# Dipet/pytorch_yolo

Measured on NVIDIA B200. Metric: YOLO decode+NMS images/sec, higher is better.
Workload: dtype f32

## Files before the change

pytorch_yolo_b200/csrc/decode.cu:

```cuda
#include <cuda.h>

#include "common.cuh"

namespace yb {

struct ScaleDev {
    const float* head;
    int ny, nx, na, row_off;
    int plane;
    int vec;
    int n_units;
    int first_block;
    int first_tile;
    int tiles_per_slab;
    float stride;
    float av[YOLO_B200_MAX_ANCHORS][2];
};

struct DecodeParams {
    ScaleDev sc[YOLO_B200_MAX_SCALES];
    int n_scales, batch, nc, rows_per_img;
    float conf, min_wh;
    yolo_b200_box* cand_box;
    yolo_b200_meta* cand_meta;
    int cap;
    int32_t* count;
    int32_t* overflow;
    float* io;
    int tp;
    int n_tiles;
    int use_tmap;
    alignas(64) CUtensorMap tmap[YOLO_B200_MAX_SCALES];
};

#ifndef YB_DC_THREADS
#define YB_DC_THREADS 128
#endif
#ifndef YB_DC_UNROLL
#define YB_DC_UNROLL 16
#endif
#ifndef YB_DC_UNROLL1
#define YB_DC_UNROLL1 40
#endif
#ifndef YB_DC_MINBLOCKS
#define YB_DC_MINBLOCKS 4
#endif
#ifndef YB_DC_SMEM_PAD
#define YB_DC_SMEM_PAD 0
#endif

constexpr int kDcThreads = YB_DC_THREADS;

template <int VEC>
__device__ __forceinline__ void load_vec(float (&dst)[VEC], const float* p) {
    if constexpr (VEC == 4) {
        const float4 v = ldg_stream4(p);
        dst[0] = v.x; dst[1] = v.y; dst[2] = v.z; dst[3] = v.w;
    } else {
        dst[0] = ldg_stream(p);
    }
}

__device__ __noinline__ void rescan_classes(const float* cls0, int stride, int nc, float& conf, int& cls) {
    float best = -1.0f;
    int bi = 0;
    for (int k = 0; k < nc; ++k) {
        const float s = sigmoidf_rn(cls0[(size_t)k * stride]);
        if (s > best) { best = s; bi = k; }
    }
    conf = best;
    cls = bi;
}

__device__ __forceinline__ void finish_anchor(const DecodeParams& P, const ScaleDev& S, bool active, int img, int a, int pos,
                                              float t0, float t1, float t2, float t3, float t4,
                                              float m, float m2, int idx, const float* cls0, int cls_stride) {
    const int nc = P.nc;
    const float stride = S.stride;
    const float conf = P.conf;
    const float kSlack = 1.00003f;
    bool emit = false;
    yolo_b200_box box = {0.f, 0.f, 0.f, 0.f};
    float score = 0.f, cls_conf = 1.0f;
    int cls = 0;
    if (active) {
        const float so = sigmoidf_rn(t4);
        const float sm = (nc > 1) ? sigmoidf_rn(m) : 1.0f;
        if (so * sm * kSlack > conf) {
            cls_conf = sm;
            cls = idx;
            if (nc > 1 && sigmoidf_rn(m2) * kSlack >= sm) rescan_classes(cls0, cls_stride, nc, cls_conf, cls);
            score = __fmul_rn(so, cls_conf);
            if (score > conf) {
                const float w = decode_wh(t2, S.av[a][0], stride);
                const float h = decode_wh(t3, S.av[a][1], stride);
                if (w > P.min_wh && h > P.min_wh && finitef(w) && finitef(h)) {
                    const int gy = pos / S.nx;
                    const int gx = pos - gy * S.nx;
                    const float x = decode_xy(t0, (float)gx, stride);
                    const float y = decode_xy(t1, (float)gy, stride);
                    if (finitef(x) && finitef(y)) {
                        emit = true;
                        box = to_corners(x, y, w, h);
                    }
                }
            }
        }
    }
    const int slot = warp_claim_slot(emit, img, P.count);
    if (emit) {
        if (slot < P.cap) {
            const int row = S.row_off + a * S.plane + pos;
            store_candidate(P.cand_box, P.cand_meta, (size_t)img * P.cap + slot, box, score, cls_conf, cls, row);
        } else {
            atomicMax(P.overflow, 1);
        }
    }
}

template <int VEC, int kDcUnroll>
__device__ __forceinline__ void decode_compact_body(const DecodeParams& P, const ScaleDev& S, int block_local) {
    const int nc = P.nc;
    const int no = nc + 5;
    const int plane = S.plane;
    const int pv_per_slab = plane / VEC;

    int unit = block_local * kDcThreads + (int)threadIdx.x;
    const bool active = unit < S.n_units;
    if (!active) unit = S.n_units - 1;
    const int slab = unit / pv_per_slab;
    const int pv = unit - slab * pv_per_slab;
    const int img = slab / S.na;
    const int a = slab - img * S.na;
    const int pos0 = pv * VEC;
    const float* base = S.head + (size_t)slab * no * plane + pos0;

    float t[5][VEC];
#pragma unroll
    for (int c = 0; c < 5; ++c) load_vec<VEC>(t[c], base + (size_t)c * plane);

    float m[VEC], m2[VEC];
    int idx[VEC];
#pragma unroll
    for (int j = 0; j < VEC; ++j) { m[j] = __int_as_float(0xff800000); m2[j] = m[j]; idx[j] = 0; }

    const float* cbase = base + (size_t)5 * plane;
    int c0 = 0;
    auto scan = [&](const float (&v)[kDcUnroll][VEC], int cfirst) {
#pragma unroll
        for (int u = 0; u < kDcUnroll; ++u) {
#pragma unroll
            for (int j = 0; j < VEC; ++j) {
                const float x = v[u][j];
                const bool up = x > m[j];
                m2[j] = up ? m[j] : fmaxf(m2[j], x);
                idx[j] = up ? (cfirst + u) : idx[j];
                m[j] = fmax_nan(m[j], x);
            }
        }
    };
    auto fetch = [&](float (&v)[kDcUnroll][VEC], int cfirst) {
#pragma unroll
        for (int u = 0; u < kDcUnroll; ++u) load_vec<VEC>(v[u], cbase + (size_t)(cfirst + u) * plane);
    };
    if (nc > 1) {
        for (; c0 + kDcUnroll <= nc; c0 += kDcUnroll) {
            float v[kDcUnroll][VEC];
            fetch(v, c0);
            scan(v, c0);
        }
        for (; c0 < nc; ++c0) {
            float v[VEC];
            load_vec<VEC>(v, cbase + (size_t)c0 * plane);
#pragma unroll
            for (int j = 0; j < VEC; ++j) {
                const float x = v[j];
                const bool up = x > m[j];
                m2[j] = up ? m[j] : fmaxf(m2[j], x);
                idx[j] = up ? c0 : idx[j];
                m[j] = fmax_nan(m[j], x);
            }
        }
    }

#pragma unroll
    for (int j = 0; j < VEC; ++j)
        finish_anchor(P, S, active, img, a, pos0 + j, t[0][j], t[1][j], t[2][j], t[3][j], t[4][j],
                      m[j], m2[j], idx[j], cbase + j, plane);
}


__global__ void __launch_bounds__(kDcThreads, YB_DC_MINBLOCKS)
decode_compact_kernel(const __grid_constant__ DecodeParams P) {
    int s = 0;
#pragma unroll
    for (int k = 1; k < YOLO_B200_MAX_SCALES; ++k)
        if (k < P.n_scales && (int)blockIdx.x >= P.sc[k].first_block) s = k;
    const ScaleDev& S = P.sc[s];
    const int block_local = (int)blockIdx.x - S.first_block;
    if (S.vec == 4) decode_compact_body<4, YB_DC_UNROLL>(P, S, block_local);
    else            decode_compact_body<1, YB_DC_UNROLL1>(P, S, block_local);
}

__device__ __forceinline__ uint32_t smem_u32(const void* p) { return (uint32_t)__cvta_generic_to_shared(p); }

__device__ __forceinline__ void mbar_init(uint64_t* bar, int count) {
    asm volatile("mbarrier.init.shared::cta.b64 [%0], %1;" ::"r"(smem_u32(bar)), "r"(count));
}
__device__ __forceinline__ void mbar_expect_tx(uint64_t* bar, uint32_t bytes) {
    asm volatile("mbarrier.arrive.expect_tx.shared::cta.b64 _, [%0], %1;" ::"r"(smem_u32(bar)), "r"(bytes) : "memory");
}
__device__ __forceinline__ void mbar_wait(uint64_t* bar, uint32_t phase) {
    asm volatile(
        "{\n\t.reg .pred p;\n\t"
        "WAIT_%=:\n\t"
        "mbarrier.try_wait.parity.shared::cta.b64 p, [%0], %1;\n\t"
        "@p bra DONE_%=;\n\t"
        "bra WAIT_%=;\n\t"
        "DONE_%=:\n\t}" ::"r"(smem_u32(bar)), "r"(phase) : "memory");
}
__device__ __forceinline__ void tma_bulk_g2s(void* dst, const void* src, uint32_t bytes, uint64_t* bar) {
    asm volatile("cp.async.bulk.shared::cluster.global.mbarrier::complete_tx::bytes [%0], [%1], %2, [%3];"
                 ::"r"(smem_u32(dst)), "l"(src), "r"(bytes), "r"(smem_u32(bar)) : "memory");
}


__device__ __forceinline__ void tma_tile_g2s(void* dst, const CUtensorMap* map, int x, int y, uint64_t* bar) {
    asm volatile("cp.async.bulk.tensor.2d.shared::cluster.global.tile.mbarrier::complete_tx::bytes [%0], [%1, {%2, %3}], [%4];"
                 ::"r"(smem_u32(dst)), "l"(map), "r"(x), "r"(y), "r"(smem_u32(bar)) : "memory");
}

constexpr int kTcConsumers = 256;
constexpr int kTcThreads = kTcConsumers + 32;
constexpr int kTcStages = 2;

__device__ __forceinline__ void mbar_arrive(uint64_t* bar) {
    asm volatile("mbarrier.arrive.shared::cta.b64 _, [%0];" ::"r"(smem_u32(bar)) : "memory");
}
__device__ __forceinline__ void consumer_bar_sync() {
    asm volatile("bar.sync 1, %0;" ::"n"(kTcConsumers) : "memory");
}

__global__ void __launch_bounds__(kTcThreads, 1)
decode_compact_tma_kernel(const __grid_constant__ DecodeParams P) {
    extern __shared__ __align__(128) float smem[];
    __shared__ __align__(8) uint64_t full[kTcStages];
    __shared__ __align__(8) uint64_t empty[kTcStages];
    const int tid = threadIdx.x;
    const int nc = P.nc, no = nc + 5, tp = P.tp;
    const int stage_floats = no * tp;

    if (tid == 0) {
#pragma unroll
        for (int s = 0; s < kTcStages; ++s) { mbar_init(&full[s], 1); mbar_init(&empty[s], kTcConsumers / 32); }
        asm volatile("fence.mbarrier_init.release.cluster;" ::: "memory");
    }
    __syncthreads();

    auto locate = [&](int tile, int& sc, int& slab, int& p0) {
        sc = 0;
#pragma unroll
        for (int k = 1; k < YOLO_B200_MAX_SCALES; ++k)
            if (k < P.n_scales && tile >= P.sc[k].first_tile) sc = k;
        const int local = tile - P.sc[sc].first_tile;
        slab = local / P.sc[sc].tiles_per_slab;
        p0 = (local - slab * P.sc[sc].tiles_per_slab) * tp;
    };

    if (tid >= kTcConsumers) {
        const int lane = tid & 31;
        int it = 0;
        for (int tile = blockIdx.x; tile < P.n_tiles; tile += gridDim.x, ++it) {
            const int st = it % kTcStages;
            mbar_wait(&empty[st], ((it / kTcStages) & 1) ^ 1);
            int sc, slab, p0;
            locate(tile, sc, slab, p0);
            const ScaleDev& S = P.sc[sc];
            if (S.vec != 4) continue;
            float* dst = smem + (size_t)st * stage_floats;
            if (P.use_tmap) {
                if (lane == 0) {
                    mbar_expect_tx(&full[st], (uint32_t)stage_floats * 4u);
                    tma_tile_g2s(dst, &P.tmap[sc], p0, slab * no, &full[st]);
                }
                continue;
            }
            const int np = min(tp, S.plane - p0);
            const uint32_t bytes = (uint32_t)np * 4u;
            if (lane == 0) mbar_expect_tx(&full[st], bytes * (uint32_t)no);
            __syncwarp();
            const float* src = S.head + (size_t)slab * no * S.plane + p0;
            for (int c = lane; c < no; c += 32)
                tma_bulk_g2s(dst + (size_t)c * tp, src + (size_t)c * S.plane, bytes, &full[st]);
        }
        return;
    }

    uint32_t full_parity = 0;
    int it = 0;
    for (int tile = blockIdx.x; tile < P.n_tiles; tile += gridDim.x, ++it) {
        const int st = it % kTcStages;
        int sc, slab, p0;
        locate(tile, sc, slab, p0);
        const ScaleDev& S = P.sc[sc];
        const int np = min(tp, S.plane - p0);
        float* tl = smem + (size_t)st * stage_floats;
        if (S.vec == 4) {
            mbar_wait(&full[st], (full_parity >> st) & 1u);
            full_parity ^= 1u << st;
        } else {
            consumer_bar_sync();
            const float* src = S.head + (size_t)slab * no * S.plane + p0;
            for (int c = tid >> 5; c < no; c += kTcConsumers / 32) {
                const float* row = src + (size_t)c * S.plane;
                float v[8];
#pragma unroll
                for (int k = 0; k < 8; ++k) { const int p = (tid & 31) + 32 * k; v[k] = p < np ? ldg_stream(row + p) : 0.0f; }
#pragma unroll
                for (int k = 0; k < 8; ++k) { const int p = (tid & 31) + 32 * k; if (p < np) tl[c * tp + p] = v[k]; }
            }
            consumer_bar_sync();
        }
        const bool active = tid < np;
        const int p = active ? tid : 0;
        const float* col = tl + p;
        const float t0 = col[0], t1 = col[tp], t2 = col[2 * tp], t3 = col[3 * tp], t4 = col[4 * tp];
        float m = __int_as_float(0xff800000), m2 = m;
        int idx = 0;
        const float* cls0 = col + 5 * tp;
        if (nc > 1) {
#pragma unroll 8
            for (int c = 0; c < nc; ++c) {
                const float x = cls0[c * tp];
                const bool up = x > m;
                m2 = up ? m : fmaxf(m2, x);
                idx = up ? c : idx;
                m = fmax_nan(m, x);
            }
        }
        const int img = slab / S.na;
        const int a = slab - img * S.na;
        finish_anchor(P, S, active, img, a, p0 + p, t0, t1, t2, t3, t4, m, m2, idx, cls0, tp);
        __syncwarp();
        if ((tid & 31) == 0) mbar_arrive(&empty[st]);
    }
}

constexpr int kDdPos = 128;
constexpr int kDdThreads = 256;
constexpr int kDdUnroll = 5;

__device__ __forceinline__ int dd_tiles_per_slab(int plane) { return (plane + kDdPos - 1) / kDdPos; }

__global__ void __launch_bounds__(kDdThreads)
decode_dense_kernel(const __grid_constant__ DecodeParams P) {
    extern __shared__ __align__(128) float smem[];
    int s = 0;
#pragma unroll
    for (int k = 1; k < YOLO_B200_MAX_SCALES; ++k)
        if (k < P.n_scales && (int)blockIdx.x >= P.sc[k].first_block) s = k;
    const ScaleDev& S = P.sc[s];
    const int nc = P.nc, no = nc + 5, plane = S.plane;
    const int tps = dd_tiles_per_slab(plane);
    const int block_local = (int)blockIdx.x - S.first_block;
    const int slab = block_local / tps;
    const int tile = block_local - slab * tps;
    const int img = slab / S.na;
    const int a = slab - img * S.na;
    const int p0 = tile * kDdPos;
    const int np = min(kDdPos, plane - p0);

    const size_t out_off = ((size_t)img * P.rows_per_img + S.row_off + (size_t)a * plane + p0) * no;
    const int mis = (int)(out_off & 3);
    float* tl = smem + mis;

    if (S.vec == 4) {
        const int warp = (int)threadIdx.x >> 5, lane = (int)threadIdx.x & 31, g = lane >> 3;
        if (4 * lane < np) {
            const float* src = S.head + (size_t)slab * no * plane + p0 + 4 * lane;
            const float stride = S.stride;
            float* drow[4];
#pragma unroll
            for (int k = 0; k < 4; ++k) drow[k] = tl + (4 * lane + ((k + g) & 3)) * no;
            auto put = [&](int ch, const float (&r)[4]) {
#pragma unroll
                for (int k = 0; k < 4; ++k) {
                    const float val = g == 0 ? r[k] : g == 1 ? r[(k + 1) & 3] : g == 2 ? r[(k + 2) & 3] : r[(k + 3) & 3];
                    drow[k][ch] = val;
                }
            };
            int c = warp;
            if (c < 4) {
                const float4 t = ldg_stream4(src + (size_t)c * plane);
                const float tv[4] = {t.x, t.y, t.z, t.w};
                float r[4];
#pragma unroll
                for (int j = 0; j < 4; ++j) {
                    const int pos = p0 + 4 * lane + j;
                    const int gy = pos / S.nx, gx = pos - gy * S.nx;
                    r[j] = c == 0 ? decode_xy(tv[j], (float)gx, stride)
                         : c == 1 ? decode_xy(tv[j], (float)gy, stride)
                                  : decode_wh(tv[j], S.av[a][c - 2], stride);
                }
                put(c, r);
                c += kDdThreads / 32;
            }
            const float* q = src + (size_t)c * plane;
            const size_t qstep = (size_t)(kDdThreads / 32) * plane;
            for (; c + (kDdUnroll - 1) * (kDdThreads / 32) < no; c += kDdUnroll * (kDdThreads / 32)) {
                float4 v[kDdUnroll];
#pragma unroll
                for (int u = 0; u < kDdUnroll; ++u, q += qstep) v[u] = ldg_stream4(q);
#pragma unroll
                for (int u = 0; u < kDdUnroll; ++u) {
                    const float r[4] = {sigmoidf_rn(v[u].x), sigmoidf_rn(v[u].y), sigmoidf_rn(v[u].z), sigmoidf_rn(v[u].w)};
                    put(c + u * (kDdThreads / 32), r);
                }
            }
            for (; c < no; c += kDdThreads / 32, q += qstep) {
                const float4 t = ldg_stream4(q);
                const float r[4] = {sigmoidf_rn(t.x), sigmoidf_rn(t.y), sigmoidf_rn(t.z), sigmoidf_rn(t.w)};
                put(c, r);
            }
            if (nc == 1 && warp == 5) {
                const float one[4] = {1.0f, 1.0f, 1.0f, 1.0f};
                put(5, one);
            }
        }
    } else {
        const int p = (int)threadIdx.x % kDdPos;
        const int half = (int)threadIdx.x / kDdPos;
        const int n_sig = no - 4;
        const int n0 = n_sig > 4 ? (n_sig - 4) / 2 : 0;
        if (p < np) {
            const float* src = S.head + (size_t)slab * no * plane + p0 + p;
            float* dst = tl + p * no;
            const float stride = S.stride;
            if (half == 0) {
                const int pos = p0 + p;
                const int gy = pos / S.nx, gx = pos - gy * S.nx;
                const float t0 = ldg_stream(src), t1 = ldg_stream(src + plane);
                const float t2 = ldg_stream(src + 2 * (size_t)plane), t3 = ldg_stream(src + 3 * (size_t)plane);
                dst[0] = decode_xy(t0, (float)gx, stride);
                dst[1] = decode_xy(t1, (float)gy, stride);
                dst[2] = decode_wh(t2, S.av[a][0], stride);
                dst[3] = decode_wh(t3, S.av[a][1], stride);
            }
            int c = half ? 4 + n0 : 4;
            const int c_end = half ? no : 4 + n0;
            const float* q = src + (size_t)c * plane;
            float* d = dst + c;
            for (; c + kDdUnroll <= c_end; c += kDdUnroll, d += kDdUnroll) {
                float v[kDdUnroll];
    #pragma unroll
                for (int u = 0; u < kDdUnroll; ++u, q += plane) v[u] = ldg_stream(q);
    #pragma unroll
                for (int u = 0; u < kDdUnroll; ++u) d[u] = sigmoidf_rn(v[u]);
            }
            for (; c < c_end; ++c, ++d, q += plane) *d = sigmoidf_rn(ldg_stream(q));
            if (nc == 1 && half == 1) dst[5] = 1.0f;
        }
    }
    __syncthreads();

    const int n_el = np * no;
    float* out = P.io + out_off;
    const int head = min(n_el, (4 - mis) & 3);
    if ((int)threadIdx.x < head) out[threadIdx.x] = tl[threadIdx.x];
    const int n4 = (n_el - head) >> 2;
    const float4* s4 = reinterpret_cast<const float4*>(tl + head);
    float4* o4 = reinterpret_cast<float4*>(out + head);
    for (int i = threadIdx.x; i < n4; i += kDdThreads) o4[i] = s4[i];
    const int done = head + (n4 << 2);
    if ((int)threadIdx.x < n_el - done) out[done + threadIdx.x] = tl[done + threadIdx.x];
}

struct DenseTmaParams {
    int stages_in, bufs_out;
};

__device__ __forceinline__ void bulk_s2g(void* gdst, const void* ssrc, uint32_t bytes) {
    asm volatile("cp.async.bulk.global.shared::cta.bulk_group [%0], [%1], %2;" ::"l"(gdst), "r"(smem_u32(ssrc)), "r"(bytes) : "memory");
}
__device__ __forceinline__ void bulk_commit() { asm volatile("cp.async.bulk.commit_group;" ::: "memory"); }
template <int N>
__device__ __forceinline__ void bulk_wait_read() { asm volatile("cp.async.bulk.wait_group.read %0;" ::"n"(N) : "memory"); }
__device__ __forceinline__ void fence_proxy_async_smem() { asm volatile("fence.proxy.async.shared::cta;" ::: "memory"); }

constexpr int kDtMaxStages = 4;

__global__ void __launch_bounds__(kTcThreads, 1)
decode_dense_tma_kernel(const __grid_constant__ DecodeParams P, const DenseTmaParams Q) {
    extern __shared__ __align__(128) float smem[];
    __shared__ __align__(8) uint64_t full[kDtMaxStages];
    __shared__ __align__(8) uint64_t empty[kDtMaxStages];
    const int tid = threadIdx.x;
    const int nc = P.nc, no = nc + 5;
    constexpr int tp = kDdPos;
    const int stage_floats = no * tp;
    const int out_floats = stage_floats + 4;
    float* out_base = smem + (size_t)Q.stages_in * stage_floats;

    if (tid == 0) {
        for (int s = 0; s < Q.stages_in; ++s) { mbar_init(&full[s], 1); mbar_init(&empty[s], kTcConsumers / 32); }
        asm volatile("fence.mbarrier_init.release.cluster;" ::: "memory");
    }
    __syncthreads();

    auto locate = [&](int tile, int& sc, int& slab, int& p0) {
        sc = 0;
#pragma unroll
        for (int k = 1; k < YOLO_B200_MAX_SCALES; ++k)
            if (k < P.n_scales && tile >= P.sc[k].first_tile) sc = k;
        const int local = tile - P.sc[sc].first_tile;
        slab = local / P.sc[sc].tiles_per_slab;
        p0 = (local - slab * P.sc[sc].tiles_per_slab) * tp;
    };

    if (tid >= kTcConsumers) {
        if ((tid & 31) != 0) return;
        int it = 0, st = 0;
        uint32_t ph = 1;
        for (int tile = blockIdx.x; tile < P.n_tiles; tile += gridDim.x, ++it) {
            mbar_wait(&empty[st], ph);
            int sc, slab, p0;
            locate(tile, sc, slab, p0);
            mbar_expect_tx(&full[st], (uint32_t)stage_floats * 4u);
            tma_tile_g2s(smem + (size_t)st * stage_floats, &P.tmap[sc], p0, slab * no, &full[st]);
            if (++st == Q.stages_in) { st = 0; ph ^= 1u; }
        }
        return;
    }

    const int p = tid & (tp - 1), half = tid >> 7;
    const int n_sig = no - 4;
    const int n0 = n_sig > 4 ? (n_sig - 4) / 2 : 0;
    uint32_t full_parity = 0;
    int it = 0, st = 0, ob = 0;
    for (int tile = blockIdx.x; tile < P.n_tiles; tile += gridDim.x, ++it) {
        int sc, slab, p0;
        locate(tile, sc, slab, p0);
        const ScaleDev& S = P.sc[sc];
        const int np = min(tp, S.plane - p0);
        const int img = slab / S.na;
        const int a = slab - img * S.na;
        float* in = smem + (size_t)st * stage_floats;
        if (tid == 0) { if (Q.bufs_out == 2) bulk_wait_read<1>(); else bulk_wait_read<0>(); }
        consumer_bar_sync();
        mbar_wait(&full[st], (full_parity >> st) & 1u);
        full_parity ^= 1u << st;

        const size_t out_off = ((size_t)img * P.rows_per_img + S.row_off + (size_t)a * S.plane + p0) * no;
        const int mis = (int)(out_off & 3);
        float* tl = out_base + (size_t)ob * out_floats + mis;
        if (p < np) {
            const float* col = in + p;
            float* dst = tl + p * no;
            const float stride = S.stride;
            if (half == 0) {
                const int pos = p0 + p;
                const int gy = pos / S.nx, gx = pos - gy * S.nx;
                dst[0] = decode_xy(col[0], (float)gx, stride);
                dst[1] = decode_xy(col[tp], (float)gy, stride);
                dst[2] = decode_wh(col[2 * tp], S.av[a][0], stride);
                dst[3] = decode_wh(col[3 * tp], S.av[a][1], stride);
            }
            int c = half ? 4 + n0 : 4;
            const int c_end = half ? no : 4 + n0;
            for (; c + 8 <= c_end; c += 8) {
                float v[8];
#pragma unroll
                for (int u = 0; u < 8; ++u) v[u] = col[(c + u) * tp];
#pragma unroll
                for (int u = 0; u < 8; ++u) dst[c + u] = sigmoidf_rn(v[u]);
            }
            for (; c < c_end; ++c) dst[c] = sigmoidf_rn(col[c * tp]);
            if (nc == 1 && half == 1) dst[5] = 1.0f;
        }
        fence_proxy_async_smem();
        __syncwarp();
        if ((tid & 31) == 0) mbar_arrive(&empty[st]);
        consumer_bar_sync();

        const int n_el = np * no;
        float* out = P.io + out_off;
        const int head = min(n_el, (4 - mis) & 3);
        const int n4 = (n_el - head) >> 2;
        const int done = head + (n4 << 2);
        if (tid == 0) {
            if (n4 > 0) bulk_s2g(out + head, tl + head, (uint32_t)n4 * 16u);
            bulk_commit();
        }
        if (tid >= 32 && tid < 32 + head) out[tid - 32] = tl[tid - 32];
        if (tid >= 64 && tid < 64 + (n_el - done)) out[done + tid - 64] = tl[done + tid - 64];

        if (++st == Q.stages_in) st = 0;
        if (++ob == Q.bufs_out) ob = 0;
    }
    if (tid == 0) bulk_wait_read<0>();
}

constexpr int kCfRows = 128;
constexpr int kCfThreads = 128;
constexpr int kCfStages = 2;

struct CompactParams {
    float* pred;
    int batch, rows_per_img, nc;
    long long total_rows;
    int n_tiles;
    int rows_tile;
    int use_tma;
    float conf, min_wh;
    int write_back;
    yolo_b200_box* cand_box;
    yolo_b200_meta* cand_meta;
    int cap;
    int32_t* count;
    int32_t* overflow;
};

__global__ void __launch_bounds__(kCfThreads)
compact_from_dense_kernel(const __grid_constant__ CompactParams P) {
    extern __shared__ __align__(128) float smem[];
    __shared__ __align__(8) uint64_t full[kCfStages];
    const int no = P.nc + 5;
    const int rows_tile = P.rows_tile;
    const int tile_floats = rows_tile * no;
    const int tid = threadIdx.x;

    if (tid == 0) {
#pragma unroll
        for (int s = 0; s < kCfStages; ++s) mbar_init(&full[s], 1);
        asm volatile("fence.mbarrier_init.release.cluster;" ::: "memory");
    }
    __syncthreads();

    auto tile_rows = [&](int t) -> int {
        const long long r0 = (long long)t * rows_tile;
        return (int)min((long long)rows_tile, P.total_rows - r0);
    };
    auto tile_is_tma = [&](int t) -> bool { return P.use_tma && tile_rows(t) == rows_tile; };
    auto issue = [&](int t, int stage) {
        if (tile_is_tma(t)) {
            const uint32_t bytes = (uint32_t)tile_floats * 4u;
            mbar_expect_tx(&full[stage], bytes);
            tma_bulk_g2s(smem + (size_t)stage * tile_floats, P.pred + (size_t)t * tile_floats, bytes, &full[stage]);
        }
    };

    uint32_t phase_bits = 0;
    int t = blockIdx.x;
    if (tid == 0) {
        int tt = t;
#pragma unroll
        for (int s = 0; s < kCfStages; ++s, tt += gridDim.x)
            if (tt < P.n_tiles) issue(tt, s);
    }
    const float inf = __int_as_float(0x7f800000);
    for (int it = 0; t < P.n_tiles; t += gridDim.x, ++it) {
        const int stage = it % kCfStages;
        float* tl = smem + (size_t)stage * tile_floats;
        const int rows = tile_rows(t);
        if (tile_is_tma(t)) {
            mbar_wait(&full[stage], (phase_bits >> stage) & 1u);
            phase_bits ^= 1u << stage;
        } else {
            const float* src = P.pred + (size_t)t * tile_floats;
            for (int i = tid; i < rows * no; i += kCfThreads) tl[i] = src[i];
            __syncthreads();
        }

        bool emit = false;
        yolo_b200_box box = {0.f, 0.f, 0.f, 0.f};
        float score = 0.f, cls_conf = 0.f;
        int cls = 0, img = 0, row = 0;
        if (tid < rows) {
            const long long g = (long long)t * rows_tile + tid;
            img = (int)(g / P.rows_per_img);
            row = (int)(g - (long long)img * P.rows_per_img);
            const float* r = tl + tid * no;
            float m = r[5], fin = __fmul_rn(r[5], 0.0f);
            int mi = 0;
            for (int k = 1; k < P.nc; ++k) {
                const float v = r[5 + k];
                fin = fmaf(v, 0.0f, fin);
                if (v > m) { m = v; mi = k; }
                m = fmax_nan(m, v);
            }
            const float x = r[0], y = r[1], w = r[2], h = r[3];
            score = __fmul_rn(r[4], m);
            if (P.write_back) P.pred[(size_t)g * no + 4] = score;
            fin = fmaf(x, 0.0f, fin); fin = fmaf(y, 0.0f, fin); fin = fmaf(w, 0.0f, fin); fin = fmaf(h, 0.0f, fin);
            fin = fmaf(score, 0.0f, fin);
            cls_conf = m;
            cls = mi;
            emit = (score > P.conf) && (w > P.min_wh) && (h > P.min_wh) && (fin == 0.0f) && (fabsf(score) < inf);
            if (emit) box = to_corners(x, y, w, h);
        }
        const int slot = warp_claim_slot(emit, img, P.count);
        if (emit) {
            if (slot < P.cap) store_candidate(P.cand_box, P.cand_meta, (size_t)img * P.cap + slot, box, score, cls_conf, cls, row);
            else atomicMax(P.overflow, 1);
        }
        __syncthreads();
        const int nt = t + kCfStages * gridDim.x;
        if (tid == 0 && nt < P.n_tiles) issue(nt, stage);
    }
}

}

using namespace yb;

static cudaError_t zero_counters(int32_t* count, int32_t* overflow, int batch, cudaStream_t stream) {
    if (overflow == count + batch) return cudaMemsetAsync(count, 0, sizeof(int32_t) * (batch + 1), stream);
    cudaError_t e = cudaSuccess;
    if (batch > 0 && (e = cudaMemsetAsync(count, 0, sizeof(int32_t) * batch, stream)) != cudaSuccess) return e;
    return cudaMemsetAsync(overflow, 0, sizeof(int32_t), stream);
}

static int fill_params(DecodeParams& P, const yolo_b200_scale* sc, int n_scales, int batch, int nc,
                       int rows_per_img, bool dense, bool partial = false) {
    if (!sc) return YOLO_B200_E_NULL;
    if (n_scales < 1 || n_scales > YOLO_B200_MAX_SCALES || batch < 0 || nc < 1 || nc > YOLO_B200_MAX_CLASSES ||
        rows_per_img < 1)
        return YOLO_B200_E_RANGE;
    const int no = nc + 5;
    long long rows = 0, blocks = 0;
    for (int k = 0; k < n_scales; ++k) {
        const yolo_b200_scale& s = sc[k];
        ScaleDev& d = P.sc[k];
        if (!s.head && batch > 0) return YOLO_B200_E_NULL;
        if (s.ny < 1 || s.nx < 1 || s.na < 1 || s.na > YOLO_B200_MAX_ANCHORS || s.row_off < 0) return YOLO_B200_E_RANGE;
        if (((uintptr_t)s.head & 3u) != 0) return YOLO_B200_E_ALIGN;
        d.head = s.head; d.ny = s.ny; d.nx = s.nx; d.na = s.na; d.row_off = s.row_off;
        d.plane = s.ny * s.nx;
        d.stride = s.stride;
        for (int a = 0; a < YOLO_B200_MAX_ANCHORS; ++a) { d.av[a][0] = s.anchor_vec[a][0]; d.av[a][1] = s.anchor_vec[a][1]; }
        d.vec = ((d.plane % 4 == 0) && (((uintptr_t)s.head & 15u) == 0)) ? 4 : 1;
        const long long slabs = (long long)batch * s.na;
        if ((long long)s.row_off + (long long)s.na * d.plane > rows_per_img) return YOLO_B200_E_RANGE;
        if (slabs * d.plane > 0x7fffffffLL) return YOLO_B200_E_RANGE;
        d.n_units = (int)(slabs * d.plane / d.vec);
        rows += (long long)s.na * d.plane;
    }
    {
        int order[YOLO_B200_MAX_SCALES];
        for (int k = 0; k < n_scales; ++k) order[k] = k;
        for (int i = 0; i < n_scales; ++i)
            for (int j = i + 1; j < n_scales; ++j) {
                const ScaleDev &a = P.sc[order[i]], &b = P.sc[order[j]];
                const bool swap = dense ? false : (b.vec > a.vec || (b.vec == a.vec && b.plane > a.plane));
                if (swap) { const int t = order[i]; order[i] = order[j]; order[j] = t; }
            }
        ScaleDev sorted[YOLO_B200_MAX_SCALES];
        for (int i = 0; i < n_scales; ++i) {
            ScaleDev& d = sorted[i];
            d = P.sc[order[i]];
            const long long slabs = (long long)batch * d.na;
            d.first_block = (int)blocks;
            if (dense) blocks += slabs * ((d.plane + kDdPos - 1) / kDdPos);
            else       blocks += (d.n_units + kDcThreads - 1) / kDcThreads;
            if (blocks > 0x7fffffffLL) return YOLO_B200_E_RANGE;
        }
        for (int i = 0; i < n_scales; ++i) P.sc[i] = sorted[i];
    }
    for (int k = n_scales; k < YOLO_B200_MAX_SCALES; ++k) { P.sc[k] = P.sc[0]; P.sc[k].first_block = 0x7fffffff; }
    if (partial ? rows > rows_per_img : rows != rows_per_img) return YOLO_B200_E_RANGE;
    P.n_scales = n_scales; P.batch = batch; P.nc = nc; P.rows_per_img = rows_per_img;
    (void)no;
    return (int)blocks;
}

static int tma_tile_positions(int no) {
    for (int tp = kTcConsumers; tp >= 32; tp >>= 1)
        if ((size_t)kTcStages * no * tp * sizeof(float) <= 200 * 1024) return tp;
    return 0;
}

static int tile_table(DecodeParams& P, int n_scales, int batch, int no, int tp, bool with_maps, bool aligned_only = false) {
    long long tiles = 0;
    P.tp = tp;
    for (int k = 0; k < n_scales; ++k) {
        P.sc[k].first_tile = (int)tiles;
        P.sc[k].tiles_per_slab = (P.sc[k].plane + tp - 1) / tp;
        if (!(aligned_only && P.sc[k].vec != 4)) tiles += (long long)batch * P.sc[k].na * P.sc[k].tiles_per_slab;
    }
    for (int k = n_scales; k < YOLO_B200_MAX_SCALES; ++k) P.sc[k].first_tile = 0x7fffffff;
    if (tiles > 0x7fffffffLL) return YOLO_B200_E_RANGE;
    P.n_tiles = (int)tiles;
    if (!with_maps) return 0;
    if (no > 256) return YOLO_B200_E_RANGE;
    typedef CUresult (*EncodeFn)(CUtensorMap*, CUtensorMapDataType, cuuint32_t, void*, const cuuint64_t*, const cuuint64_t*,
                                 const cuuint32_t*, const cuuint32_t*, CUtensorMapInterleave, CUtensorMapSwizzle,
                                 CUtensorMapL2promotion, CUtensorMapFloatOOBfill);
    void* fn = nullptr;
    cudaDriverEntryPointQueryResult qres;
    const cudaError_t e = cudaGetDriverEntryPoint("cuTensorMapEncodeTiled", &fn, cudaEnableDefault, &qres);
    if (e != cudaSuccess) return (int)e;
    if (!fn || qres != cudaDriverEntryPointSuccess) return YOLO_B200_E_RANGE;
    for (int k = 0; k < n_scales; ++k) {
        if (P.sc[k].vec != 4) continue;
        const cuuint64_t gdim[2] = {(cuuint64_t)P.sc[k].plane, (cuuint64_t)batch * P.sc[k].na * no};
        const cuuint64_t gstride[1] = {(cuuint64_t)P.sc[k].plane * sizeof(float)};
        const cuuint32_t box[2] = {(cuuint32_t)tp, (cuuint32_t)no};
        const cuuint32_t estr[2] = {1, 1};
        const CUresult r = ((EncodeFn)fn)(&P.tmap[k], CU_TENSOR_MAP_DATA_TYPE_FLOAT32, 2, (void*)P.sc[k].head, gdim, gstride,
                                          box, estr, CU_TENSOR_MAP_INTERLEAVE_NONE, CU_TENSOR_MAP_SWIZZLE_NONE,
                                          CU_TENSOR_MAP_L2_PROMOTION_L2_256B, CU_TENSOR_MAP_FLOAT_OOB_FILL_NONE);
        if (r != CUDA_SUCCESS) return YOLO_B200_E_RANGE;
    }
    return 0;
}

extern "C" int yolo_b200_decode_compact_ex(const yolo_b200_scale* scales, int n_scales, int batch, int nc,
                                           int rows_per_img, float conf_thres, float min_wh,
                                           yolo_b200_box* cand_box, yolo_b200_meta* cand_meta, int cap_per_img,
                                           int32_t* count, int32_t* overflow, int variant, yolo_b200_stream_t stream) {
    if (!cand_box || !cand_meta || !count || !overflow) return YOLO_B200_E_NULL;
    const bool accumulate = variant >= 0 && (variant & YOLO_B200_VARIANT_ACCUMULATE) != 0;
    if (accumulate) variant &= ~YOLO_B200_VARIANT_ACCUMULATE;
    if (cap_per_img < 1 || variant < 0 || variant > 3) return YOLO_B200_E_RANGE;
    if ((((uintptr_t)cand_box) | ((uintptr_t)cand_meta)) & 15u) return YOLO_B200_E_ALIGN;
    DecodeParams P{};
    const int blocks = fill_params(P, scales, n_scales, batch, nc, rows_per_img, false, accumulate);
    if (blocks < 0) return blocks;
    P.conf = conf_thres; P.min_wh = min_wh;
    P.cand_box = cand_box; P.cand_meta = cand_meta; P.cap = cap_per_img; P.count = count; P.overflow = overflow;
    cudaError_t e;
    if (!accumulate && (e = zero_counters(count, overflow, batch, stream)) != cudaSuccess) return (int)e;
    if (blocks == 0) return 0;

    int dev = 0, sms = 148;
    if (cudaGetDevice(&dev) == cudaSuccess) cudaDeviceGetAttribute(&sms, cudaDevAttrMultiProcessorCount, dev);
    const int no = nc + 5;
    const int tp = tma_tile_positions(no);
    const bool use_tma = tp > 0 && variant >= 2;
    if (variant >= 2 && tp == 0) return YOLO_B200_E_RANGE;
    P.use_tmap = 0;
    if (use_tma) {
        const int rc = tile_table(P, n_scales, batch, no, tp, variant == 3);
        if (rc != 0) return rc;
        P.use_tmap = variant == 3 ? 1 : 0;
    }
    const long long tiles = P.n_tiles;
    if (use_tma) {
        const size_t smem = (size_t)kTcStages * no * tp * sizeof(float);
        if ((e = cudaFuncSetAttribute(decode_compact_tma_kernel, cudaFuncAttributeMaxDynamicSharedMemorySize, (int)smem)) != cudaSuccess)
            return (int)e;
        const int grid = (int)(tiles < sms ? tiles : sms);
        decode_compact_tma_kernel<<<grid, kTcThreads, smem, stream>>>(P);
    } else {
        decode_compact_kernel<<<blocks, kDcThreads, YB_DC_SMEM_PAD, stream>>>(P);
    }
    return (int)cudaGetLastError();
}

extern "C" int yolo_b200_decode_compact(const yolo_b200_scale* scales, int n_scales, int batch, int nc,
                                        int rows_per_img, float conf_thres, float min_wh,
                                        yolo_b200_box* cand_box, yolo_b200_meta* cand_meta, int cap_per_img,
                                        int32_t* count, int32_t* overflow, yolo_b200_stream_t stream) {
    return yolo_b200_decode_compact_ex(scales, n_scales, batch, nc, rows_per_img, conf_thres, min_wh, cand_box, cand_meta,
                                       cap_per_img, count, overflow, 0, stream);
}

extern "C" int yolo_b200_decode_dense_ex(const yolo_b200_scale* scales, int n_scales, int batch, int nc,
                                         int rows_per_img, float* io, int variant, yolo_b200_stream_t stream) {
    if (!io) return YOLO_B200_E_NULL;
    if ((uintptr_t)io & 15u) return YOLO_B200_E_ALIGN;
    if (variant < 0 || variant > 2) return YOLO_B200_E_RANGE;
    DecodeParams P{};
    const int blocks = fill_params(P, scales, n_scales, batch, nc, rows_per_img, true);
    if (blocks < 0) return blocks;
    P.io = io;
    if (blocks == 0) return 0;
    const int no = nc + 5;
    const size_t tile_bytes = (size_t)kDdPos * no * sizeof(float);
    cudaError_t e;
    bool any_aligned = false;
    for (int k = 0; k < n_scales; ++k) any_aligned |= P.sc[k].vec == 4;
    const size_t budget = 226 * 1024;
    DenseTmaParams Q{0, 0};
    if (no <= 256 && any_aligned) {
        if (5 * tile_bytes + 32 <= budget)      Q = {3, 2};
        else if (4 * tile_bytes + 32 <= budget) Q = {2, 2};
        else if (3 * tile_bytes + 16 <= budget) Q = {2, 1};
    }
    if (variant == 2 && Q.stages_in == 0) return YOLO_B200_E_RANGE;
    const size_t ldg_smem = tile_bytes + 4 * sizeof(float);
    if (ldg_smem > 220 * 1024) return YOLO_B200_E_RANGE;
    if ((e = cudaFuncSetAttribute(decode_dense_kernel, cudaFuncAttributeMaxDynamicSharedMemorySize, (int)ldg_smem)) != cudaSuccess)
        return (int)e;
    if (variant != 1 && Q.stages_in > 0) {
        const int rc = tile_table(P, n_scales, batch, no, kDdPos, true, true);
        if (rc != 0) return rc;
        const size_t smem = (size_t)Q.stages_in * tile_bytes + (size_t)Q.bufs_out * (tile_bytes + 16);
        if ((e = cudaFuncSetAttribute(decode_dense_tma_kernel, cudaFuncAttributeMaxDynamicSharedMemorySize, (int)smem)) != cudaSuccess)
            return (int)e;
        int dev = 0, sms = 148;
        if (cudaGetDevice(&dev) == cudaSuccess) cudaDeviceGetAttribute(&sms, cudaDevAttrMultiProcessorCount, dev);
        const int grid = P.n_tiles < sms ? P.n_tiles : sms;
        decode_dense_tma_kernel<<<grid, kTcThreads, smem, stream>>>(P, Q);
        if ((e = cudaGetLastError()) != cudaSuccess) return (int)e;
        long long rest = 0;
        for (int k = 0; k < n_scales; ++k) {
            P.sc[k].first_block = (int)rest;
            if (P.sc[k].vec != 4) rest += (long long)batch * P.sc[k].na * ((P.sc[k].plane + kDdPos - 1) / kDdPos);
        }
        if (rest == 0) return 0;
        decode_dense_kernel<<<(int)rest, kDdThreads, ldg_smem, stream>>>(P);
        return (int)cudaGetLastError();
    }
    decode_dense_kernel<<<blocks, kDdThreads, ldg_smem, stream>>>(P);
    return (int)cudaGetLastError();
}

extern "C" int yolo_b200_decode_dense(const yolo_b200_scale* scales, int n_scales, int batch, int nc,
                                      int rows_per_img, float* io, yolo_b200_stream_t stream) {
    return yolo_b200_decode_dense_ex(scales, n_scales, batch, nc, rows_per_img, io, 0, stream);
}

extern "C" int yolo_b200_compact_from_dense(float* pred, int batch, int rows_per_img, int nc,
                                            float conf_thres, float min_wh, int write_back_score,
                                            yolo_b200_box* cand_box, yolo_b200_meta* cand_meta, int cap_per_img,
                                            int32_t* count, int32_t* overflow, yolo_b200_stream_t stream) {
    if (!cand_box || !cand_meta || !count || !overflow || (!pred && batch > 0)) return YOLO_B200_E_NULL;
    if (batch < 0 || rows_per_img < 1 || nc < 1 || nc > YOLO_B200_MAX_CLASSES || cap_per_img < 1) return YOLO_B200_E_RANGE;
    if (((uintptr_t)pred & 3u) || ((((uintptr_t)cand_box) | ((uintptr_t)cand_meta)) & 15u)) return YOLO_B200_E_ALIGN;
    CompactParams P{};
    P.pred = pred; P.batch = batch; P.rows_per_img = rows_per_img; P.nc = nc;
    P.total_rows = (long long)batch * rows_per_img;
    int rows_tile = kCfRows;
    while (rows_tile > 4 && (size_t)kCfStages * rows_tile * (nc + 5) * sizeof(float) > 200 * 1024) rows_tile >>= 1;
    P.rows_tile = rows_tile;
    const long long tiles = (P.total_rows + rows_tile - 1) / rows_tile;
    if (tiles > 0x7fffffffLL) return YOLO_B200_E_RANGE;
    P.n_tiles = (int)tiles;
    P.use_tma = (((uintptr_t)pred & 15u) == 0) ? 1 : 0;
    P.conf = conf_thres; P.min_wh = min_wh; P.write_back = write_back_score;
    P.cand_box = cand_box; P.cand_meta = cand_meta; P.cap = cap_per_img; P.count = count; P.overflow = overflow;
    cudaError_t e;
    if ((e = zero_counters(count, overflow, batch, stream)) != cudaSuccess) return (int)e;
    if (P.n_tiles == 0) return 0;
    const size_t smem = (size_t)kCfStages * rows_tile * (nc + 5) * sizeof(float);
    if (smem > 200 * 1024) return YOLO_B200_E_RANGE;
    if ((e = cudaFuncSetAttribute(compact_from_dense_kernel, cudaFuncAttributeMaxDynamicSharedMemorySize, (int)smem)) != cudaSuccess)
        return (int)e;
    int dev = 0, sms = 148;
    if (cudaGetDevice(&dev) == cudaSuccess) cudaDeviceGetAttribute(&sms, cudaDevAttrMultiProcessorCount, dev);
    const int per_sm = (int)((220 * 1024) / (smem + 1024));
    const int grid = (int)min((long long)sms * (per_sm < 1 ? 1 : per_sm), tiles);
    compact_from_dense_kernel<<<grid, kCfThreads, smem, stream>>>(P);
    return (int)cudaGetLastError();
}
```

Baseline: 765,900.

## Gate decode on objectness and compact passing units before class scan

```diff
diff --git a/profiles/gate_sweep.py b/profiles/gate_sweep.py
--- /dev/null
+++ b/profiles/gate_sweep.py
@@ -0,0 +1,81 @@
+import glob
+import os
+import statistics
+import sys
+
+import torch
+
+ROOT = os.path.dirname(os.path.dirname(os.path.abspath(__file__)))
+sys.path.insert(0, ROOT)
+from pytorch_yolo_b200 import _lib, ops, synth
+
+CONFIGS = [("cfg2 spp-608 b64 conf 0.3", "spp-608", 64, 0.3), ("cfg4 spp-608 b64 conf 0.001", "spp-608", 64, 0.001),
+           ("cfg3 tiny-416 b1024 conf 0.3", "tiny-416", 1024, 0.3), ("cfg5 spp-1024 b256 conf 0.3", "spp-1024", 256, 0.3)]
+
+
+def use(path):
+    os.environ["YOLO_B200_LIB"] = path
+    _lib._lib = None
+    _lib.load()
+
+
+def candidates(buf, rows_per_img):
+    B, cap = buf.batch, buf.cap
+    meta = buf.meta[:B + 1].clone()
+    count = meta[:B].clamp(max=cap).long()
+    slot = torch.arange(cap, device=buf.meta.device)
+    valid = (slot[None, :] < count[:, None]).reshape(-1)
+    img = torch.arange(B, device=buf.meta.device).repeat_interleave(cap)[valid]
+    m = buf.cand_meta[:B * cap][valid]
+    bx = buf.cand_box[:B * cap][valid].view(torch.int32)
+    key = img * rows_per_img + m[:, 3].long()
+    order = torch.argsort(key)
+    return meta.cpu(), torch.cat([bx, m], 1)[order].cpu()
+
+
+def main():
+    rounds = int(sys.argv[1]) if len(sys.argv) > 1 else 5
+    launches = int(sys.argv[2]) if len(sys.argv) > 2 else 50
+    libs = sorted(glob.glob(os.path.join(ROOT, "build", "variants", "*.so")))
+    names = [os.path.basename(p)[:-3] for p in libs]
+    dev = "cuda:0"
+    print(f"device {torch.cuda.get_device_name(0)}; {rounds} rounds x {launches} launches per library and config", flush=True)
+    for label, wl, B, conf in CONFIGS:
+        w = synth.WORKLOADS[wl]
+        heads = synth.synth_heads(wl, B, "B", seed=1234, device=dev)
+        specs = [ops.scale_spec(a, g, g, w["img_size"]) for a, g in zip(w["anchors"], w["grids"])]
+        rows = synth.anchors_per_image(wl)
+        use(libs[0])
+        buf = ops.Buffers(dev, B, rows, w["nc"])
+        times = {n: [] for n in names}
+        results = {}
+        for rnd in range(rounds):
+            for path, name in zip(libs, names):
+                use(path)
+                for _ in range(5):
+                    ops.decode_compact(heads, specs, w["nc"], conf, buf, variant="ldg")
+                torch.cuda.synchronize()
+                if rnd == 0:
+                    results[name] = candidates(buf, rows)
+                e0, e1 = torch.cuda.Event(enable_timing=True), torch.cuda.Event(enable_timing=True)
+                e0.record()
+                for _ in range(launches):
+                    ops.decode_compact(heads, specs, w["nc"], conf, buf, variant="ldg")
+                e1.record()
+                torch.cuda.synchronize()
+                times[name].append(e0.elapsed_time(e1) / launches * 1000.0)
+        nbytes = B * synth.head_bytes_per_image(wl)
+        ref = results.get("parent")
+        print(f"\n{label}: {nbytes / 1e6:.1f} MB per launch, {int(results[names[0]][0][:B].sum())} candidates", flush=True)
+        print(f"  {'library':12s} {'median us':>10s} {'min':>8s} {'max':>8s} {'dense-eq TB/s':>14s}  same as parent")
+        for n in names:
+            t = times[n]
+            same = "-" if ref is None else str(torch.equal(results[n][0], ref[0]) and torch.equal(results[n][1], ref[1]))
+            print(f"  {n:12s} {statistics.median(t):10.1f} {min(t):8.1f} {max(t):8.1f} {nbytes / statistics.median(t) / 1e6:14.2f}  {same}",
+                  flush=True)
+        del heads, buf
+        torch.cuda.empty_cache()
+
+
+if __name__ == "__main__":
+    main()
diff --git a/profiles/gate_traffic.py b/profiles/gate_traffic.py
--- /dev/null
+++ b/profiles/gate_traffic.py
@@ -0,0 +1,55 @@
+import os
+import sys
+
+import torch
+
+ROOT = os.path.dirname(os.path.dirname(os.path.abspath(__file__)))
+sys.path.insert(0, ROOT)
+from pytorch_yolo_b200 import synth
+
+CONFIGS = [("cfg2 spp-608 b64 conf 0.3", "spp-608", 64, 0.3), ("cfg5 spp-1024 b256 conf 0.3", "spp-1024", 256, 0.3),
+           ("cfg3 tiny-416 b1024 conf 0.3", "tiny-416", 1024, 0.3), ("cfg4 spp-608 b64 conf 0.001", "spp-608", 64, 0.001)]
+
+
+def traffic(workload, batch, conf, granules):
+    w = synth.WORKLOADS[workload]
+    no = w["nc"] + 5
+    heads = synth.synth_heads(workload, batch, "B", seed=1234)
+    dense = 0
+    fetched = {g: 0 for g in granules}
+    n_pass = n_pos = n_quads = n_quads_pass = 0
+    for h, anchors in zip(heads, w["anchors"]):
+        B, _, gy, gx = h.shape
+        na, plane = len(anchors), gy * gx
+        obj = torch.sigmoid(h.view(B, na, no, plane)[:, :, 4, :]) > conf
+        n_pass += int(obj.sum())
+        n_pos += obj.numel()
+        dense += h.numel() * 4
+        m = obj.reshape(B * na, plane)
+        if plane % 4 == 0:
+            q = m.view(B * na, plane // 4, 4).any(2)
+            n_quads_pass += int(q.sum())
+            n_quads += q.numel()
+        slab, p = m.nonzero(as_tuple=True)
+        for g in granules:
+            fetched[g] += B * na * plane * 4
+            for c in range(no):
+                if c != 4:
+                    addr = ((slab * no + c) * plane + p) * 4
+                    fetched[g] += int(torch.unique(addr // g).numel()) * g
+    return n_pass / n_pos, (n_quads_pass / n_quads if n_quads else float("nan")), dense, fetched
+
+
+def main():
+    granules = [int(a) for a in sys.argv[1:]] or [32, 64, 128]
+    torch.set_num_threads(min(8, os.cpu_count() or 1))
+    print(f"{'config':30s} {'pass':>7s} {'quads':>7s} {'dense MB':>9s} " +
+          " ".join(f"{f'{g} B: fetched MB, / dense, predicted us':>40s}" for g in granules))
+    for label, wl, b, conf in CONFIGS:
+        fp, fq, dense, fetched = traffic(wl, b, conf, granules)
+        cols = " ".join(f"{fetched[g] / 1e6:20.1f} {fetched[g] / dense:8.3f} {10 + fetched[g] / 5.9e6:10.1f}" for g in granules)
+        print(f"{label:30s} {fp:7.4f} {fq:7.4f} {dense / 1e6:9.1f} {cols}", flush=True)
+
+
+if __name__ == "__main__":
+    main()
diff --git a/profiles/sector_granularity_probe.cu b/profiles/sector_granularity_probe.cu
--- /dev/null
+++ b/profiles/sector_granularity_probe.cu
@@ -0,0 +1,99 @@
+#include <cuda_runtime.h>
+
+#include <algorithm>
+#include <cstdio>
+#include <cstdlib>
+#include <vector>
+
+#define CK(x) do { cudaError_t e_ = (x); if (e_ != cudaSuccess) { std::printf("%s: %s\n", #x, cudaGetErrorString(e_)); std::exit(1); } } while (0)
+
+__device__ __forceinline__ float4 ldg_stream4(const float4* p) {
+    float4 v;
+    asm volatile("ld.global.nc.L1::no_allocate.v4.f32 {%0,%1,%2,%3}, [%4];" : "=f"(v.x), "=f"(v.y), "=f"(v.z), "=f"(v.w) : "l"(p));
+    return v;
+}
+
+constexpr int kInFlight = 8;
+
+template <int MODE>
+__global__ void __launch_bounds__(256) probe(const float4* buf, long long n_lines, float* sink) {
+    const long long nth = (long long)gridDim.x * blockDim.x;
+    const long long n_units = MODE == 0 ? n_lines * 8 : n_lines;
+    float acc = 0.f;
+    for (long long u0 = (long long)blockIdx.x * blockDim.x + threadIdx.x; u0 < n_units; u0 += nth * kInFlight) {
+        float4 v[kInFlight][2];
+#pragma unroll
+        for (int k = 0; k < kInFlight; ++k) {
+            const long long u = u0 + k * nth;
+            if (u < n_units) {
+                if (MODE == 0) { v[k][0] = ldg_stream4(buf + u); v[k][1] = make_float4(0.f, 0.f, 0.f, 0.f); }
+                else {
+                    v[k][0] = ldg_stream4(buf + u * 8);
+                    v[k][1] = MODE == 1 ? make_float4(0.f, 0.f, 0.f, 0.f) : ldg_stream4(buf + u * 8 + (MODE == 2 ? 2 : 4));
+                }
+            } else {
+                v[k][0] = v[k][1] = make_float4(0.f, 0.f, 0.f, 0.f);
+            }
+        }
+#pragma unroll
+        for (int k = 0; k < kInFlight; ++k) acc += v[k][0].x + v[k][0].w + v[k][1].y + v[k][1].z;
+    }
+    if (acc == 1234567.f) sink[0] = acc;
+}
+
+template <int MODE>
+static float time_pattern(const float4* buf, long long n_lines, float* sink, int grid, int reps) {
+    cudaEvent_t a, b;
+    CK(cudaEventCreate(&a));
+    CK(cudaEventCreate(&b));
+    for (int i = 0; i < 3; ++i) probe<MODE><<<grid, 256>>>(buf, n_lines, sink);
+    CK(cudaDeviceSynchronize());
+    std::vector<float> ms;
+    for (int i = 0; i < reps; ++i) {
+        CK(cudaEventRecord(a));
+        probe<MODE><<<grid, 256>>>(buf, n_lines, sink);
+        CK(cudaEventRecord(b));
+        CK(cudaEventSynchronize(b));
+        float t;
+        CK(cudaEventElapsedTime(&t, a, b));
+        ms.push_back(t);
+    }
+    CK(cudaGetLastError());
+    std::sort(ms.begin(), ms.end());
+    CK(cudaEventDestroy(a));
+    CK(cudaEventDestroy(b));
+    return ms[ms.size() / 2];
+}
+
+int main(int argc, char** argv) {
+    const double gib = argc > 1 ? std::atof(argv[1]) : 4.0;
+    const size_t bytes = (size_t)(gib * (1ull << 30)) / 128 * 128;
+    const long long n_lines = (long long)(bytes / 128);
+    cudaDeviceProp prop;
+    CK(cudaGetDeviceProperties(&prop, 0));
+    float4* buf;
+    float* sink;
+    CK(cudaMalloc(&buf, bytes));
+    CK(cudaMalloc(&sink, sizeof(float)));
+    CK(cudaMemset(buf, 0, bytes));
+    const int grid = prop.multiProcessorCount * 8;
+    const int reps = 30;
+    std::printf("device %s, %d SMs, L2 %d MB; buffer %.2f GB; grid %d x 256 threads, %d loads in flight per thread; "
+                "median of %d launches\n", prop.name, prop.multiProcessorCount, prop.l2CacheSize >> 20, bytes / 1e9, grid,
+                kInFlight, reps);
+    const float t0 = time_pattern<0>(buf, n_lines, sink, grid, reps);
+    const float t1 = time_pattern<1>(buf, n_lines, sink, grid, reps);
+    const float t2 = time_pattern<2>(buf, n_lines, sink, grid, reps);
+    const float t3 = time_pattern<3>(buf, n_lines, sink, grid, reps);
+    struct { const char* name; float ms; int sectors; } rows[] = {
+        {"dense (4 of 4 sectors)", t0, 4}, {"1 of 4 sectors per line", t1, 1},
+        {"2 of 4, same 64 B half", t2, 2}, {"2 of 4, one per 64 B", t3, 2}};
+    std::printf("%-26s %10s %10s %14s %22s\n", "pattern", "ms", "vs dense", "requested GB/s", "line-equivalent GB/s");
+    for (auto& r : rows)
+        std::printf("%-26s %10.3f %10.3f %14.1f %22.1f\n", r.name, r.ms, r.ms / t0, bytes * (r.sectors / 4.0) / (r.ms * 1e6),
+                    bytes / (r.ms * 1e6));
+    std::printf("effective granule from '1 of 4': %.0f B; from '2 of 4 split': %.0f B per 64 B\n", t1 / t0 * 128.0, t3 / t0 * 64.0);
+    CK(cudaFree(buf));
+    CK(cudaFree(sink));
+    return 0;
+}
diff --git a/profiles/summarize_alternated.py b/profiles/summarize_alternated.py
--- /dev/null
+++ b/profiles/summarize_alternated.py
@@ -0,0 +1,23 @@
+import json
+import statistics
+import sys
+
+
+def main():
+    rows = [json.loads(line) for line in open(sys.argv[1]) if line.strip()]
+    configs = list(dict.fromkeys(r["config"] for r in rows))
+    builds = list(dict.fromkeys(r["build"] for r in rows))
+    for c in configs:
+        base = None
+        for b in builds:
+            sel = [r["line"] for r in rows if r["config"] == c and r["build"] == b]
+            v = [x["value"] for x in sel]
+            us = [x["ms_per_step"] * 1000 for x in sel]
+            med = statistics.median(v)
+            base = base or med
+            print(f"{c:9s} {b:7s} median {med:10.0f} images/s ({med / base:5.3f}x)  range {min(v):.0f}-{max(v):.0f}  "
+                  f"us/step {[round(x, 1) for x in us]}")
+
+
+if __name__ == "__main__":
+    main()
diff --git a/profiles/trace_step.py b/profiles/trace_step.py
--- /dev/null
+++ b/profiles/trace_step.py
@@ -0,0 +1,60 @@
+import collections
+import json
+import os
+import sys
+
+import torch
+
+ROOT = os.path.dirname(os.path.dirname(os.path.abspath(__file__)))
+sys.path.insert(0, ROOT)
+import bench
+
+
+def main():
+    out_dir = sys.argv[1]
+    steps = int(sys.argv[2]) if len(sys.argv) > 2 else 10
+    os.makedirs(out_dir, exist_ok=True)
+    c = bench.Case("spp-608", 64, "B", 0.3, 0.5, torch.device("cuda:0"), 0, 1)
+    c.run_steps(300)
+    torch.cuda.synchronize()
+    path = os.path.join(out_dir, "r03_c_step_trace.pt.trace.json")
+    with torch.profiler.profile(activities=[torch.profiler.ProfilerActivity.CPU, torch.profiler.ProfilerActivity.CUDA]) as prof:
+        c.run_steps(steps)
+        torch.cuda.synchronize()
+    prof.export_chrome_trace(path)
+    with open(path) as f:
+        ev = [e for e in json.load(f)["traceEvents"] if e.get("cat") == "kernel"]
+    ev.sort(key=lambda e: e["ts"])
+    t0, t1 = ev[0]["ts"], max(e["ts"] + e["dur"] for e in ev)
+    print(f"device {torch.cuda.get_device_name(0)}; {steps} steps traced; {len(ev)} kernels; "
+          f"first kernel start -> last kernel end {t1 - t0:.1f} us = {(t1 - t0) / steps:.1f} us per step")
+    per = collections.defaultdict(list)
+    for e in ev:
+        per[(e["name"][:60], e["args"].get("stream"))].append(e["dur"])
+    print(f"{'kernel':60s} {'stream':>6s} {'count':>6s} {'mean us':>8s} {'min':>7s} {'max':>7s}")
+    for (name, stream), d in sorted(per.items(), key=lambda kv: -sum(kv[1])):
+        print(f"{name:60s} {str(stream):>6s} {len(d):6d} {sum(d) / len(d):8.1f} {min(d):7.1f} {max(d):7.1f}")
+    busy, gaps, end = 0.0, [], t0
+    for e in ev:
+        s, f = e["ts"], e["ts"] + e["dur"]
+        if s > end:
+            gaps.append(s - end)
+        busy += max(0.0, f - max(s, end))
+        end = max(end, f)
+    print(f"busy {busy:.1f} us of {t1 - t0:.1f} us ({busy / (t1 - t0):.3f}); {len(gaps)} gaps with no kernel running, "
+          f"total {sum(gaps):.1f} us, largest {max(gaps) if gaps else 0:.1f} us")
+    dec = [e for e in ev if "decode_compact_kernel" in e["name"]]
+    if dec:
+        ov = 0.0
+        for d in dec:
+            s, f = d["ts"], d["ts"] + d["dur"]
+            for e in ev:
+                if e is not d and e["ts"] < f and e["ts"] + e["dur"] > s:
+                    ov += min(f, e["ts"] + e["dur"]) - max(s, e["ts"])
+        print(f"decode_compact_kernel: {len(dec)} launches, mean {sum(d['dur'] for d in dec) / len(dec):.1f} us; "
+              f"other kernels running beside it: {ov / len(dec):.1f} us per launch (kernel-time sum)")
+    c.close()
+
+
+if __name__ == "__main__":
+    main()
diff --git a/pytorch_yolo_b200/csrc/decode.cu b/pytorch_yolo_b200/csrc/decode.cu
--- a/pytorch_yolo_b200/csrc/decode.cu
+++ b/pytorch_yolo_b200/csrc/decode.cu
@@ -49,7 +49,13 @@
 #define YB_DC_SMEM_PAD 0
 #endif
 
+#ifndef YB_DC_GATE_R
+#define YB_DC_GATE_R 2
+#endif
+
 constexpr int kDcThreads = YB_DC_THREADS;
+constexpr int kDcGateR = YB_DC_GATE_R;
+constexpr int kDcChunk = kDcThreads * kDcGateR;
 
 template <int VEC>
 __device__ __forceinline__ void load_vec(float (&dst)[VEC], const float* p) {
@@ -119,15 +125,12 @@
 }
 
 template <int VEC, int kDcUnroll>
-__device__ __forceinline__ void decode_compact_body(const DecodeParams& P, const ScaleDev& S, int block_local) {
+__device__ __forceinline__ void decode_compact_unit(const DecodeParams& P, const ScaleDev& S, int unit, bool active) {
     const int nc = P.nc;
     const int no = nc + 5;
     const int plane = S.plane;
     const int pv_per_slab = plane / VEC;
 
-    int unit = block_local * kDcThreads + (int)threadIdx.x;
-    const bool active = unit < S.n_units;
-    if (!active) unit = S.n_units - 1;
     const int slab = unit / pv_per_slab;
     const int pv = unit - slab * pv_per_slab;
     const int img = slab / S.na;
@@ -187,6 +190,61 @@
     for (int j = 0; j < VEC; ++j)
         finish_anchor(P, S, active, img, a, pos0 + j, t[0][j], t[1][j], t[2][j], t[3][j], t[4][j],
                       m[j], m2[j], idx[j], cbase + j, plane);
+}
+
+__device__ __forceinline__ bool gate_pass(float t4, float conf) {
+    return __fmul_rn(sigmoidf_rn(t4), 1.0f + 1.0f / 4194304.0f) > conf;
+}
+
+template <int VEC, int kDcUnroll>
+__device__ __forceinline__ void decode_compact_body(const DecodeParams& P, const ScaleDev& S, int block_local) {
+    constexpr int kWarps = kDcThreads / 32;
+    __shared__ int wcount[kDcGateR][kWarps];
+    __shared__ unsigned short list[kDcChunk];
+    const int tid = (int)threadIdx.x, lane = tid & 31, warp = tid >> 5;
+    const int no = P.nc + 5, plane = S.plane, pv_per_slab = plane / VEC;
+    const int base = block_local * kDcChunk;
+
+    float o[kDcGateR][VEC];
+#pragma unroll
+    for (int r = 0; r < kDcGateR; ++r) {
+        const int unit = base + r * kDcThreads + tid;
+        if (unit < S.n_units) {
+            const int slab = unit / pv_per_slab;
+            load_vec<VEC>(o[r], S.head + ((size_t)slab * no + 4) * plane + (size_t)(unit - slab * pv_per_slab) * VEC);
+        } else {
+#pragma unroll
+            for (int j = 0; j < VEC; ++j) o[r][j] = __int_as_float(0x7fffffff);
+        }
+    }
+    unsigned mask[kDcGateR];
+#pragma unroll
+    for (int r = 0; r < kDcGateR; ++r) {
+        bool pass = false;
+#pragma unroll
+        for (int j = 0; j < VEC; ++j) pass |= gate_pass(o[r][j], P.conf);
+        mask[r] = __ballot_sync(kFull, pass);
+        if (lane == 0) wcount[r][warp] = __popc(mask[r]);
+    }
+    __syncthreads();
+    int n = 0;
+#pragma unroll
+    for (int r = 0; r < kDcGateR; ++r) {
+        int off = n;
+#pragma unroll
+        for (int w = 0; w < kWarps; ++w) {
+            const int c = wcount[r][w];
+            off += w < warp ? c : 0;
+            n += c;
+        }
+        if ((mask[r] >> lane) & 1u) list[off + __popc(mask[r] & ((1u << lane) - 1u))] = (unsigned short)(r * kDcThreads + tid);
+    }
+    __syncthreads();
+    for (int k = warp * 32; k < n; k += kDcThreads) {
+        const int item = k + lane;
+        const bool active = item < n;
+        decode_compact_unit<VEC, kDcUnroll>(P, S, base + list[active ? item : k], active);
+    }
 }
 
 
@@ -743,6 +801,7 @@
         if ((long long)s.row_off + (long long)s.na * d.plane > rows_per_img) return YOLO_B200_E_RANGE;
         if (slabs * d.plane > 0x7fffffffLL) return YOLO_B200_E_RANGE;
         d.n_units = (int)(slabs * d.plane / d.vec);
+        if (d.n_units + (long long)kDcChunk > 0x7fffffffLL) return YOLO_B200_E_RANGE;
         rows += (long long)s.na * d.plane;
     }
     {
@@ -761,7 +820,7 @@
             const long long slabs = (long long)batch * d.na;
             d.first_block = (int)blocks;
             if (dense) blocks += slabs * ((d.plane + kDdPos - 1) / kDdPos);
-            else       blocks += (d.n_units + kDcThreads - 1) / kDcThreads;
+            else       blocks += (d.n_units + kDcChunk - 1) / kDcChunk;
             if (blocks > 0x7fffffffLL) return YOLO_B200_E_RANGE;
         }
         for (int i = 0; i < n_scales; ++i) P.sc[i] = sorted[i];
```

After: 904,200, median of 6. 1.18x the previous value.
